# PantoMatrix/PantoMatrix

Hardware: NVIDIA H100
Metric: motion_frames_per_sec (higher is better)
Workload: dtype fp16x3 (two fp16 operand planes, 3 products, f32 accumulate)

## Files before the change

### include/pm_emage.h

```cpp
#ifndef PM_EMAGE_H
#define PM_EMAGE_H
#include <stdint.h>
#ifdef __cplusplus
extern "C" {
#endif

#define PM_ABI_VERSION 6
#define PM_FMT_F16 0x100
#define PM_TC_TILE_SHIFT 16
#define PM_TC_STORE_LOOP (1 << 24)
int pm_abi_version(void);
int pm_memset_async(void* ptr, int value, long long bytes, void* stream);
int pm_device_cc(void);

int pm_tapgemm_f32(const float* A, long long a_bs, int lda, int batch, int rows_in, int cin,
                   const float* W, const float* bias, int taps, int stride, int pad,
                   int rows_out, int cout,
                   const float* residual, long long r_bs, int ldr,
                   int act, float slope,
                   float* out, long long o_bs, int ldo, void* stream);

int pm_tapgemm_tc(const uint16_t* A, long long a_ps, long long a_bs, int lda, int batch, int rows_in, int cin,
                  const uint16_t* W, long long w_ps, int w_rows, int ldw, int taps, int pad, int nsplit,
                  const float* bias, int rows_out, int cout,
                  const float* residual, long long r_bs, int ldr,
                  int act, int act_cols, float slope, float acc_scale,
                  float* out_f32, long long o_bs, int ldo,
                  uint16_t* out_bf16, long long ob_ps, long long ob_bs, int ldob, int out_nsplit,
                  const void* prefetch, long long prefetch_bytes, void* stream);

int pm_split_bf16(const float* x, long long x_bs, int ldx, int batch, int rows, int ch,
                  uint16_t* out, long long o_ps, long long o_bs, int ldo, int nsplit, void* stream);

int pm_wav_stem_f32(const float* audio, long long a_bs, long long a_ws, int batch, int windows, int n_samples,
                    const float* w1, const float* b1, const float* wd, const float* bd, int cout,
                    int ksize, int stride, int pad, int rows_out, float slope,
                    float* y1, float* sc,
                    uint16_t* planes, long long p_ps, int p_ld, int p_nsplit, void* stream);

int pm_add_layernorm_f32(const float* x, const float* r, const float* gamma, const float* beta,
                         float* out, long long rows, int ch, float eps,
                         uint16_t* planes, long long p_ps, int p_ld, int p_nsplit, void* stream);

// ... 110 lines not shown
```

### pantomatrix_b200/csrc/pm_tapgemm_tc.cu

```cuda
#include <cuda.h>
#include <stdio.h>
#include <stdlib.h>

#include <cstring>
#include <type_traits>
#include "pm_common.cuh"
#include "../../include/pm_emage.h"


namespace {

constexpr int BM = 128;
constexpr int BK = 64;
constexpr int MMA_K = 16;
constexpr int A_TILE_BYTES = BM * BK * 2;
constexpr int PRODUCER_THREADS = 128;
constexpr int CONSUMER_THREADS = 256;
constexpr int NUM_THREADS = PRODUCER_THREADS + CONSUMER_THREADS;
constexpr int PRODUCER_REGS = 40, CONSUMER_REGS = 232;
static_assert(PRODUCER_THREADS * PRODUCER_REGS + CONSUMER_THREADS * CONSUMER_REGS == (65536 / NUM_THREADS & ~7) * NUM_THREADS,
              "the setmaxnreg split must use exactly the launch's register pool");
constexpr int STAMP_WARP = PRODUCER_THREADS / 32;
constexpr int MAX_STAGES = 8;
constexpr int RING_KB = 200;

struct TcParams {
  int taps, pad, nsplit, kblocks;
  int rows_out, cout, batch;
  int R, NB;
  int w_rows;
  const float* bias;
  const float* residual; long long r_bs; int ldr;
  int res_tma;
  int tma_out;
  int act, act_cols; float slope;
  float* out_f32; long long o_bs; int ldo;
  __nv_bfloat16* out_bf16; long long ob_ps, ob_bs; int ldob; int out_nsplit;
  int stages;
  int res_slot0, rot;
  const uint8_t* prefetch; long long prefetch_bytes;
  float acc_scale;
};

#ifdef PM_TC_TIMING
__device__ unsigned long long pm_tc_stamps[4096 * 8];
#define PM_STAMP(i)                                                                                              \
  do {                                                                                                           \
    if ((threadIdx.x & 31) == 0) {                                                                               \
      const unsigned cta_ = (blockIdx.z * gridDim.y + blockIdx.y) * gridDim.x + blockIdx.x;                      \
      if (cta_ < 4096) pm_tc_stamps[cta_ * 8 + (i)] = (unsigned long long)clock64();                             \
    }                                                                                                            \
  } while (0)
#else
#define PM_STAMP(i) do {} while (0)
#endif

#include "pm_tc_ptx.cuh"

template <int BN, bool F16>
__device__ __forceinline__ void mma_k16(float (&d)[BN / 2], uint64_t a, uint64_t b) {
  static_assert(BN == 64 || BN == 128, "64- or 128-column tiles (see pm_tapgemm_tc)");
  if constexpr (BN == 64) wgmma_m64n64k16<!F16>(d, a, b);
  else wgmma_m64n128k16<!F16>(d, a, b);
}

template <int BN, bool F16, int NSPLIT>
__device__ __forceinline__ void mma_kblock(float (&main)[BN / 2], float (&corr)[BN / 2], uint64_t a0, uint64_t w0) {
  constexpr uint64_t A_PL = A_TILE_BYTES >> 4, W_PL = (BN * BK * 2) >> 4, K_ST = (MMA_K * 2) >> 4;
  if constexpr (NSPLIT == 3) {
#pragma unroll
    for (int k = 0; k < BK / MMA_K; ++k) mma_k16<BN, F16>(corr, a0 + k * K_ST, w0 + 2 * W_PL + k * K_ST);
#pragma unroll
    for (int k = 0; k < BK / MMA_K; ++k) mma_k16<BN, F16>(corr, a0 + A_PL + k * K_ST, w0 + W_PL + k * K_ST);
#pragma unroll
    for (int k = 0; k < BK / MMA_K; ++k) mma_k16<BN, F16>(corr, a0 + 2 * A_PL + k * K_ST, w0 + k * K_ST);
  }
  if constexpr (NSPLIT >= 2) {
#pragma unroll
    for (int k = 0; k < BK / MMA_K; ++k) mma_k16<BN, F16>(corr, a0 + k * K_ST, w0 + W_PL + k * K_ST);
#pragma unroll
    for (int k = 0; k < BK / MMA_K; ++k) mma_k16<BN, F16>(corr, a0 + A_PL + k * K_ST, w0 + k * K_ST);
  }
#pragma unroll
  for (int k = 0; k < BK / MMA_K; ++k) mma_k16<BN, F16>(main, a0 + k * K_ST, w0 + k * K_ST);
}

template <int BN, bool F16, int NSPLIT>
__global__ void __launch_bounds__(NUM_THREADS, 1) tapgemm_tc_kernel(const __grid_constant__ CUtensorMap map_a,
                                                                  const __grid_constant__ CUtensorMap map_w,
                                                                  const __grid_constant__ CUtensorMap map_r,
                                                                  const __grid_constant__ CUtensorMap map_o,
                                                                  const __grid_constant__ CUtensorMap map_p,
                                                                  const TcParams p) {
  constexpr int W_TILE_BYTES = BN * BK * 2;
  constexpr int NACC = BN / 2;
  constexpr int ST = BN + 8;
  constexpr int RES_BYTES = BM * BN * 4;

  extern __shared__ __align__(1024) uint8_t smem_raw[];
  uint8_t* tiles = smem_raw + ((1024u - (smem_u32(smem_raw) & 1023u)) & 1023u);
  const int stage_bytes = p.nsplit * (A_TILE_BYTES + W_TILE_BYTES);
  const int ring_bytes = p.stages * stage_bytes > BM * ST * 4 ? p.stages * stage_bytes : BM * ST * 4;
  uint64_t* bars = reinterpret_cast<uint64_t*>(tiles + ring_bytes);
  uint64_t* full_bar = bars;
  uint64_t* empty_bar = bars + MAX_STAGES;
  uint64_t* epi_bar = bars + 2 * MAX_STAGES;
  float* bias_s = reinterpret_cast<float*>(bars + 2 * MAX_STAGES + 2);

  const int warp = threadIdx.x >> 5, lane = threadIdx.x & 31;
  if (warp == STAMP_WARP) PM_STAMP(0);
  const int l0 = blockIdx.x * p.R;
  const int n0 = blockIdx.y * BN;
  const int b0 = blockIdx.z * p.NB;
  const int n_iter = p.taps * p.kblocks;

  if (threadIdx.x == 0) {
    asm volatile("prefetch.tensormap [%0];" ::"l"(&map_a) : "memory");
    asm volatile("prefetch.tensormap [%0];" ::"l"(&map_w) : "memory");
    if (p.res_tma) asm volatile("prefetch.tensormap [%0];" ::"l"(&map_r) : "memory");
    if (p.tma_out && p.out_f32) asm volatile("prefetch.tensormap [%0];" ::"l"(&map_o) : "memory");
    if (p.tma_out && p.out_nsplit) asm volatile("prefetch.tensormap [%0];" ::"l"(&map_p) : "memory");
    for (int s = 0; s < p.stages; ++s) {
      mbar_init(smem_u32(&full_bar[s]), 1);
      mbar_init(smem_u32(&empty_bar[s]), 2);
    }
    mbar_init(smem_u32(epi_bar), p.res_tma ? 2 : 1);
    asm volatile("fence.mbarrier_init.release.cluster;" ::: "memory");
  }
  __syncthreads();
  if (warp == STAMP_WARP) PM_STAMP(1);

  if (warp < PRODUCER_THREADS / 32) {
    setmaxnreg_dec<PRODUCER_REGS>();
    if (warp == 1 && lane == 0 && p.prefetch) {
      const long long ncta = (long long)gridDim.x * gridDim.y * gridDim.z;
      const long long cta = ((long long)blockIdx.z * gridDim.y + blockIdx.y) * gridDim.x + blockIdx.x;
      long long share = ((p.prefetch_bytes + ncta - 1) / ncta + 127) & ~127LL;
      long long off = cta * share;
      long long end = off + share < p.prefetch_bytes ? off + share : p.prefetch_bytes;
      end &= ~15LL;
      for (; off < end; off += 16384) {
        const uint32_t n = (uint32_t)(end - off < 16384 ? end - off : 16384);
        asm volatile("cp.async.bulk.prefetch.L2.global [%0], %1;" ::"l"(p.prefetch + off), "r"(n) : "memory");
      }
    }
    if (warp == 2) {
      for (int c = lane; c < BN; c += 32) bias_s[c] = p.bias && n0 + c < p.cout ? __ldg(p.bias + n0 + c) : 0.f;
      __syncwarp();
      if (lane == 0) mbar_arrive(smem_u32(epi_bar));
    }
    if (warp != 0) return;
    const uint32_t tx = (uint32_t)stage_bytes;
    int s = 0, q = p.rot, tap = 0, kb = 0;
    uint32_t ph = 0;
    for (int it = 0; it < n_iter; ++it) {
      mbar_wait_fast(smem_u32(&empty_bar[s]), ph ^ 1u);
      if (elect_one()) {
        const uint32_t bar = smem_u32(&full_bar[s]);
        uint8_t* st = tiles + (size_t)q * stage_bytes;
        mbar_expect_tx(bar, tx);
        for (int pl = 0; pl < p.nsplit; ++pl) {
          tma_load_4d(smem_u32(st + pl * A_TILE_BYTES), &map_a, bar, kb * BK, l0 + tap - p.pad, b0, pl);
          tma_load_3d(smem_u32(st + p.nsplit * A_TILE_BYTES + pl * W_TILE_BYTES), &map_w, bar, kb * BK, tap * p.w_rows + n0, pl);
        }
      }
      __syncwarp();
      if (++s == p.stages) { s = 0; ph ^= 1u; }
      if (++q == p.stages) q = 0;
      if (++kb == p.kblocks) { kb = 0; ++tap; }
    }
    if (p.res_tma) {
      for (int j = p.res_slot0; j < p.stages; ++j) {
        mbar_wait_fast(smem_u32(&empty_bar[s]), ph ^ 1u);
        if (++s == p.stages) { s = 0; ph ^= 1u; }
      }
      if (elect_one()) {
        const uint32_t bar = smem_u32(epi_bar);
        mbar_expect_tx(bar, (uint32_t)RES_BYTES);
        const int nbox = p.tma_out ? BN / 32 : 1;
        for (int j = 0; j < nbox; ++j)
          tma_load_3d(smem_u32(tiles + ring_bytes - RES_BYTES + j * (RES_BYTES / nbox)), &map_r, bar, n0 + j * (BN / nbox), l0, b0);
      }
      __syncwarp();
    }
    return;
  }

  setmaxnreg_inc<CONSUMER_REGS>();
  const int ct = threadIdx.x - PRODUCER_THREADS;
  const int wg = ct >> 7;
  float acc0[NACC], acc1[NACC], accc[NACC];
#pragma unroll
  for (int i = 0; i < NACC; ++i) { acc0[i] = 0.f; acc1[i] = 0.f; accc[i] = 0.f; }
  {
    const uint32_t tiles_u32 = smem_u32(tiles);
    int s = 0, q = p.rot;
    uint32_t ph = 0;
    int prev = -1;
    auto kblock = [&](float (&main)[NACC]) {
      mbar_wait_fast(smem_u32(&full_bar[s]), ph);
      if (prev < 0 && warp == STAMP_WARP) PM_STAMP(2);
      const uint32_t a_base = tiles_u32 + (uint32_t)q * (uint32_t)stage_bytes + (uint32_t)wg * (64 * 128);
      const uint32_t w_base = tiles_u32 + (uint32_t)q * (uint32_t)stage_bytes + (uint32_t)(NSPLIT * A_TILE_BYTES);
      wgmma_fence();
      mma_kblock<BN, F16, NSPLIT>(main, accc, gmma_desc(GMMA_DESC_K_SW128, a_base), gmma_desc(GMMA_DESC_K_SW128, w_base));
      wgmma_commit();
      wgmma_wait<1>();
      if (prev >= 0 && ct % 128 == 0) mbar_arrive(smem_u32(&empty_bar[prev]));
      prev = s;
      if (++s == p.stages) { s = 0; ph ^= 1u; }
      if (++q == p.stages) q = 0;
    };
    int it = 0;
    for (; it + 1 < n_iter; it += 2) {
      kblock(acc0);
      kblock(acc1);
    }
    if (it < n_iter) kblock(acc0);
    if (warp == STAMP_WARP) PM_STAMP(3);
    wgmma_wait<0>();
    if (warp == STAMP_WARP) PM_STAMP(4);
    wgmma_fence_regs(acc0);
    wgmma_fence_regs(acc1);
    wgmma_fence_regs(accc);
  }
  named_bar_sync(1, CONSUMER_THREADS);
  if (p.tma_out) {
    const int wq = warp & 3, t4 = lane & 3, sw = lane >> 2;
    const int r0 = wg * 64 + wq * 16 + sw;
    const float act_slope = p.act == PM_ACT_NONE ? 1.f : (p.act == PM_ACT_RELU ? 0.f : p.slope);
    const float* res_s = reinterpret_cast<const float*>(tiles + ring_bytes - RES_BYTES);
    auto off32 = [&](int r, int i) { return (i >> 2) * (BM * 32) + r * 32 + (((2 * (i & 3) + (t4 >> 1)) ^ sw) << 2) + 2 * (t4 & 1); };
    mbar_wait_fast(smem_u32(epi_bar), 0);
#pragma unroll
    for (int i = 0; i < NACC / 4; ++i) {
      const int c = 8 * i + 2 * t4, n = n0 + c;
      const float2 bc = *reinterpret_cast<const float2*>(bias_s + c);
#pragma unroll
      for (int h = 0; h < 2; ++h) {
        const int j = 4 * i + 2 * h;
        float v0 = acc0[j] + acc1[j], v1 = acc0[j + 1] + acc1[j + 1];
        v0 += accc[j];
        v1 += accc[j + 1];
        if constexpr (F16) { v0 = __fmul_rn(v0, p.acc_scale); v1 = __fmul_rn(v1, p.acc_scale); }
// ... 133 lines not shown
}

template <bool VEC, bool F16>
__global__ void __launch_bounds__(256) split_bf16_kernel(const float* __restrict__ x, long long x_bs, int ldx, int rows,
                                                         int ch, __nv_bfloat16* __restrict__ out, long long o_ps,
                                                         long long o_bs, int ldo, int nsplit) {
  const int b = blockIdx.y;
  const float* __restrict__ xb = x + (long long)b * x_bs;
  __nv_bfloat16* __restrict__ ob = out + (long long)b * o_bs;
  if (VEC) {
    const int ch4 = ch >> 2;
    const long long total = (long long)rows * ch4;
    for (long long i = (long long)blockIdx.x * blockDim.x + threadIdx.x; i < total; i += (long long)gridDim.x * blockDim.x) {
      const int r = (int)(i / ch4), c4 = (int)(i - (long long)r * ch4);
      const float4 v = *reinterpret_cast<const float4*>(xb + (long long)r * ldx + 4 * c4);
      const PmPlanes P{ob, o_ps, ldo, nsplit};
      pm_store_planes4_t<F16>(P, r, 4 * c4, v);
    }
  } else {
    const long long total = (long long)rows * ch;
    for (long long i = (long long)blockIdx.x * blockDim.x + threadIdx.x; i < total; i += (long long)gridDim.x * blockDim.x) {
      const int r = (int)(i / ch), c = (int)(i - (long long)r * ch);
      const PmPlanes P{ob, o_ps, ldo, nsplit};
      pm_store_planes_t<F16>(P, r, c, xb[(long long)r * ldx + c]);
    }
  }
}

constexpr int stage_bytes_of(int bn, int nsplit) { return nsplit * (A_TILE_BYTES + bn * BK * 2); }
constexpr int stages_of(int bn, int nsplit) {
  return RING_KB * 1024 / stage_bytes_of(bn, nsplit) < MAX_STAGES ? RING_KB * 1024 / stage_bytes_of(bn, nsplit) : MAX_STAGES;
}
constexpr int ring_bytes_of(int bn, int nsplit) { return stages_of(bn, nsplit) * stage_bytes_of(bn, nsplit); }
constexpr bool tma_out_fits(int bn, int nsplit, bool f32, int out_nsplit, bool residual) {
  return (f32 ? BM * bn * 4 : 0) + out_nsplit * BM * bn * 2 + (residual ? BM * bn * 4 : 0) <= ring_bytes_of(bn, nsplit);
}

template <int BN, bool F16, int NSPLIT>
int launch(const CUtensorMap& ma, const CUtensorMap& mw, const CUtensorMap& mr, const CUtensorMap& mo,
           const CUtensorMap& mp, TcParams& p, dim3 grid, cudaStream_t st) {
  constexpr int stage_bytes = stage_bytes_of(BN, NSPLIT);
  constexpr int stages = stages_of(BN, NSPLIT);
  static_assert(stages >= 2, "the operand ring needs two stages");
  constexpr int staging = BM * (BN + 8) * 4, res_bytes = BM * BN * 4;
  static_assert(staging + res_bytes <= stages * stage_bytes && res_bytes <= (stages - 1) * stage_bytes,
                "staging and residual tiles must fit the ring side by side");
  static_assert(tma_out_fits(BN, NSPLIT, true, 2, true), "fp32, two plane and residual tiles must fit the ring");
  static_assert(BN * 4 * BM % 1024 == 0 && stage_bytes % 1024 == 0, "128B-swizzled TMA boxes need 1024-byte alignment");
  p.stages = stages;
  p.res_slot0 = (stages * stage_bytes - res_bytes) / stage_bytes;
  p.rot = (p.res_slot0 - 1 - (p.taps * p.kblocks - 1) % stages + stages) % stages;
  const size_t smem = (size_t)stages * stage_bytes + 1024  + (2 * MAX_STAGES + 2) * sizeof(uint64_t) + BN * sizeof(float);
  static unsigned long long configured = 0;
  if (pm_first_use_on_device(configured)) {
    cudaError_t e = cudaFuncSetAttribute(tapgemm_tc_kernel<BN, F16, NSPLIT>, cudaFuncAttributeMaxDynamicSharedMemorySize, 227 * 1024);
    if (e != cudaSuccess) { configured = 0; return (int)e; }
  }
  tapgemm_tc_kernel<BN, F16, NSPLIT><<<grid, NUM_THREADS, smem, st>>>(ma, mw, mr, mo, mp, p);
  PM_LAUNCH_CHECK();
}

template <int BN>
int launch_fmt(const CUtensorMap* m, TcParams& p, dim3 grid, cudaStream_t st, bool f16) {
  if (f16) {
    if (p.nsplit == 1) return launch<BN, true, 1>(m[0], m[1], m[2], m[3], m[4], p, grid, st);
    if (p.nsplit == 2) return launch<BN, true, 2>(m[0], m[1], m[2], m[3], m[4], p, grid, st);
    return launch<BN, true, 3>(m[0], m[1], m[2], m[3], m[4], p, grid, st);
  }
  if (p.nsplit == 1) return launch<BN, false, 1>(m[0], m[1], m[2], m[3], m[4], p, grid, st);
  if (p.nsplit == 2) return launch<BN, false, 2>(m[0], m[1], m[2], m[3], m[4], p, grid, st);
  return launch<BN, false, 3>(m[0], m[1], m[2], m[3], m[4], p, grid, st);
}

int pick_bn(long long row_tiles, int cout, int w_rows, int sms) {
  if (cout <= 64 || w_rows % 128) return 64;
  const long long waves64 = (row_tiles * pm_cdiv(cout, 64) + sms - 1) / sms;
  const long long waves128 = (row_tiles * pm_cdiv(cout, 128) + sms - 1) / sms;
  return waves128 * 14 <= waves64 * 10 ? 128 : 64;
}

}

extern "C" int pm_tapgemm_tc(const uint16_t* A, long long a_ps, long long a_bs, int lda, int batch, int rows_in, int cin,
                             const uint16_t* W, long long w_ps, int w_rows, int ldw, int taps, int pad, int nsplit,
                             const float* bias, int rows_out, int cout,
                             const float* residual, long long r_bs, int ldr,
                             int act, int act_cols, float slope, float acc_scale,
                             float* out_f32, long long o_bs, int ldo,
                             uint16_t* out_bf16, long long ob_ps, long long ob_bs, int ldob, int out_nsplit,
                             const void* prefetch, long long prefetch_bytes, void* stream) {
  PM_REQUIRE(A && W && (out_f32 || out_bf16));
  const int tile = (nsplit >> PM_TC_TILE_SHIFT) & 0xff;
  const bool store_loop = (nsplit & PM_TC_STORE_LOOP) != 0;
  PM_TAKE_FMT(nsplit, f16);
  PM_TAKE_FMT(out_nsplit, out_f16);
  PM_REQUIRE(!out_bf16 || out_f16 == f16);
  PM_REQUIRE(f16 || acc_scale == 1.0f);
  PM_REQUIRE(!prefetch || (prefetch_bytes >= 0 && (reinterpret_cast<uintptr_t>(prefetch) & 15) == 0));
  PM_REQUIRE(batch > 0 && rows_in > 0 && rows_out > 0 && cin > 0 && cout > 0 && taps > 0);
  PM_REQUIRE(nsplit >= 1 && nsplit <= 3 && (!out_bf16 || (out_nsplit >= 1 && out_nsplit <= 3)));
  PM_REQUIRE(act >= PM_ACT_NONE && act <= PM_ACT_LEAKY);
  PM_REQUIRE((reinterpret_cast<uintptr_t>(A) & 15) == 0 && (reinterpret_cast<uintptr_t>(W) & 15) == 0);
  PM_REQUIRE((lda & 7) == 0 && (ldw & 7) == 0 && lda >= cin && ldw >= cin && w_rows >= cout);
  PM_REQUIRE(batch == 1 || (a_bs & 7) == 0);
  PM_REQUIRE(nsplit == 1 || ((a_ps & 7) == 0 && (w_ps & 7) == 0));
  PM_REQUIRE(!out_f32 || ldo >= cout);
  PM_REQUIRE(!out_bf16 || ldob >= cout);
  PM_REQUIRE(!residual || ldr >= cout);

  int R = 128;
  if (rows_out <= 64 && batch > 1) { R = 16; while (R < rows_out) R <<= 1; }
  const int NB = 128 / R;
  PM_REQUIRE(tile <= 2 && w_rows % 64 == 0 && (tile != 2 || w_rows % 128 == 0));
  int BNsel = tile == 1 ? 64 : 128;
  if (tile == 0) {
    int dev = 0, sms = 0;
    cudaError_t e = cudaGetDevice(&dev);
    if (e == cudaSuccess) e = cudaDeviceGetAttribute(&sms, cudaDevAttrMultiProcessorCount, dev);
    if (e != cudaSuccess) return (int)e;
    BNsel = pick_bn((long long)pm_cdiv(rows_out, R) * pm_cdiv(batch, NB), cout, w_rows, sms);
  }

  TcParams p;
  p.taps = taps; p.pad = pad; p.nsplit = nsplit; p.kblocks = (cin + BK - 1) / BK;
  p.rows_out = rows_out; p.cout = cout; p.batch = batch; p.R = R; p.NB = NB; p.w_rows = w_rows;
  p.bias = bias; p.residual = residual; p.r_bs = r_bs; p.ldr = ldr;
  p.act = act; p.act_cols = act_cols <= 0 ? cout : act_cols; p.slope = slope;
  p.out_f32 = out_f32; p.o_bs = o_bs; p.ldo = ldo;
  p.out_bf16 = reinterpret_cast<__nv_bfloat16*>(out_bf16); p.ob_ps = ob_ps; p.ob_bs = ob_bs; p.ldob = ldob;
  p.out_nsplit = out_bf16 ? out_nsplit : 0;
  p.stages = 0;
  p.prefetch = static_cast<const uint8_t*>(prefetch);
  p.prefetch_bytes = prefetch ? prefetch_bytes : 0;
  p.acc_scale = acc_scale;
  CUtensorMap m[5];
  std::memset(m, 0, sizeof(m));
  CUtensorMap &ma = m[0], &mw = m[1], &mr = m[2], &mo = m[3], &mp = m[4];
  {
    const long long bs_el = batch > 1 ? a_bs : (long long)rows_in * lda;
    const long long ps_el = nsplit > 1 ? a_ps : bs_el * batch;
    cuuint64_t dims[4] = {(cuuint64_t)cin, (cuuint64_t)rows_in, (cuuint64_t)batch, (cuuint64_t)nsplit};
    cuuint64_t strides[3] = {(cuuint64_t)lda * 2, (cuuint64_t)bs_el * 2, (cuuint64_t)ps_el * 2};
    cuuint32_t box[4] = {(cuuint32_t)BK, (cuuint32_t)R, (cuuint32_t)NB, 1};
    if (!encode_map(&ma, A, 4, dims, strides, box, f16)) return PM_EBADARG;
  }
  {
    const long long ps_el = nsplit > 1 ? w_ps : (long long)taps * w_rows * ldw;
    cuuint64_t dims[3] = {(cuuint64_t)cin, (cuuint64_t)taps * w_rows, (cuuint64_t)nsplit};
    cuuint64_t strides[2] = {(cuuint64_t)ldw * 2, (cuuint64_t)ps_el * 2};
    cuuint32_t box[3] = {(cuuint32_t)BK, (cuuint32_t)BNsel, 1};
    if (!encode_map(&mw, W, 3, dims, strides, box, f16)) return PM_EBADARG;
  }
  const bool res_ok = residual && (reinterpret_cast<uintptr_t>(residual) & 15) == 0 && (ldr & 3) == 0 && (batch == 1 || (r_bs & 3) == 0);
  bool tma_out = !store_loop && (!residual || res_ok) && tma_out_fits(BNsel, nsplit, out_f32, p.out_nsplit, residual);
  if (tma_out && out_f32) {
    tma_out = (reinterpret_cast<uintptr_t>(out_f32) & 15) == 0 && (ldo & 3) == 0 && (batch == 1 || (o_bs & 3) == 0);
    const long long bs_el = batch > 1 ? o_bs : (long long)rows_out * ldo;
    cuuint64_t dims[3] = {(cuuint64_t)cout, (cuuint64_t)rows_out, (cuuint64_t)batch};
    cuuint64_t strides[2] = {(cuuint64_t)ldo * 4, (cuuint64_t)bs_el * 4};
    cuuint32_t box[3] = {32, (cuuint32_t)R, (cuuint32_t)NB};
    tma_out = tma_out && encode_tiled(&mo, CU_TENSOR_MAP_DATA_TYPE_FLOAT32, CU_TENSOR_MAP_SWIZZLE_128B, out_f32, 3, dims, strides, box);
  }
  if (tma_out && out_bf16) {
    tma_out = (reinterpret_cast<uintptr_t>(out_bf16) & 15) == 0 && (ldob & 7) == 0 && (batch == 1 || (ob_bs & 7) == 0) &&
              (out_nsplit == 1 || (ob_ps & 7) == 0);
    const long long bs_el = batch > 1 ? ob_bs : (long long)rows_out * ldob;
    const long long ps_el = out_nsplit > 1 ? ob_ps : bs_el * batch;
    cuuint64_t dims[4] = {(cuuint64_t)cout, (cuuint64_t)rows_out, (cuuint64_t)batch, (cuuint64_t)out_nsplit};
    cuuint64_t strides[3] = {(cuuint64_t)ldob * 2, (cuuint64_t)bs_el * 2, (cuuint64_t)ps_el * 2};
    cuuint32_t box[4] = {64, (cuuint32_t)R, (cuuint32_t)NB, 1};
    tma_out = tma_out && encode_map(&mp, out_bf16, 4, dims, strides, box, f16);
  }
  p.res_tma = false;
  for (int swz = tma_out; res_ok && !p.res_tma && swz >= 0; --swz) {
    const long long bs_el = batch > 1 ? r_bs : (long long)rows_out * ldr;
    cuuint64_t dims[3] = {(cuuint64_t)cout, (cuuint64_t)rows_out, (cuuint64_t)batch};
    cuuint64_t strides[2] = {(cuuint64_t)ldr * 4, (cuuint64_t)bs_el * 4};
    cuuint32_t box[3] = {swz ? 32u : (cuuint32_t)BNsel, (cuuint32_t)R, (cuuint32_t)NB};
    p.res_tma = encode_tiled(&mr, CU_TENSOR_MAP_DATA_TYPE_FLOAT32, swz ? CU_TENSOR_MAP_SWIZZLE_128B : CU_TENSOR_MAP_SWIZZLE_NONE,
                             residual, 3, dims, strides, box);
    if (!p.res_tma) tma_out = false;
  }
  p.tma_out = tma_out;
  dim3 grid(pm_cdiv(rows_out, R), pm_cdiv(cout, BNsel), pm_cdiv(batch, NB));
  PM_REQUIRE(grid.z <= 65535 && grid.y <= 65535);
  const cudaStream_t st = (cudaStream_t)stream;
  if (BNsel == 128) return launch_fmt<128>(m, p, grid, st, f16);
// ... 44 lines not shown
```

### pantomatrix_b200/emage_audio/engine.py

```python
from __future__ import annotations

import os

import torch

from .. import ops

PARTS = ("face", "upper", "hands", "lower")
WAV_BLOCKS = ((5, 1600, True), (6, 0, True), (1, 7, False), (6, 0, True), (1, 7, False), (3, 0, True))
NHEAD = 4


def _taps(w: torch.Tensor) -> torch.Tensor:
    return w.permute(2, 0, 1).contiguous()


def _fold_bn(sd, conv, bn, eps=1e-5):
    w, b = sd[conv + ".weight"].double(), sd[conv + ".bias"].double()
    s = sd[bn + ".weight"].double() / torch.sqrt(sd[bn + ".running_var"].double() + eps)
    return (w * s[:, None, None]).float(), ((b - sd[bn + ".running_mean"].double()) * s + sd[bn + ".bias"].double()).float()


def wav_out_len(n: int) -> int:
    length = n
# ... 95 lines not shown
            _record_stream(results[i], cur)
        return results


class _Conv:
    __slots__ = ("w", "b", "stride", "pad", "_packed", "_next")

    def __init__(self, w, b, stride=1, pad=0):
        self.w, self.b, self.stride, self.pad = w, b, stride, pad
        self._packed = {}
        self._next = None

    def _prefetch_hint(self, ns):
        prev = _STATE.get("prev_conv")
        if prev is not None and prev is not self:
            prev._next = self
        _STATE["prev_conv"] = self
        nxt = self._next
        return nxt._packed[_pk(ns)].t if (nxt is not None and _pk(ns) in nxt._packed) else None

    def packed(self, nsplit):
        key = _pk(nsplit)
        if key not in self._packed:
            w, s = self.w, self.stride
            if s > 1:
                taps, cout, cin = w.shape
                wp = torch.zeros(-(-taps // s), cout, s * cin, device=w.device, dtype=w.dtype)
                for k in range(taps):
                    wp[k // s, :, (k % s) * cin:(k % s + 1) * cin] = w[k]
                w = wp
            self._packed[key] = ops.PackedW(w, nsplit)
        return self._packed[key]

    def __call__(self, x, act=ops.ACT_NONE, slope=0.0, residual=None, out=None, want="f", out_slack=0):
        ns = _STATE["nsplit"]
        residual = _f32(residual)
        if ns == 0:
            y = ops.tapgemm(_f32(x), self.w, self.b, stride=self.stride, pad=self.pad, act=act, slope=slope,
                            residual=residual, out=out)
            return y if want == "f" else ops.Act(y, None)
        taps, cout, _ = self.w.shape
        s = self.stride
        want_f, out_ns = "f" in want, (ns if "p" in want else 0)
        pf = self._prefetch_hint(ns)
        if s == 1:
            a = _planes(x, ns)
            batch, rows = a.batch, a.rows
            rows_out = rows + 2 * self.pad - taps + 1
            flat = (taps == 1 and batch > 1 and a.t.stride(1) == rows * a.t.stride(2)
                    and (out is None or out.is_contiguous()) and (residual is None or residual.is_contiguous()))
            if want_f and out is None:
                out = torch.empty(batch, rows_out, cout, device=a.t.device, dtype=torch.float32)
            if flat:
                _, pl = ops.tapgemm_tc(a.flat(), self.packed(ns), self.b, rows_out=batch * rows, act=act, slope=slope,
                                       want_f32=want_f, out=None if out is None else out.view(1, batch * rows, cout),
                                       residual=None if residual is None else residual.view(1, batch * rows, cout),
                                       out_nsplit=out_ns, out_slack=out_slack, prefetch=pf)
                if pl is not None:
                    pl = ops.Planes(pl.t.view(pl.t.shape[0], batch, rows, pl.t.shape[3]), rows, cout, pl.slack)
            else:
                _, pl = ops.tapgemm_tc(a, self.packed(ns), self.b, rows_out=rows_out, pad=self.pad, act=act, slope=slope,
                                       residual=residual, want_f32=want_f, out=out, out_nsplit=out_ns, out_slack=out_slack,
                                       prefetch=pf)
            return out if want == "f" else ops.Act(out, pl)
        assert self.pad == 0
        a = _planes(x, ns, need_slack=s)
        batch, rows, cin = a.batch, a.rows, a.ch
        assert a.t.stride(2) == cin and a.t.stride(1) == rows * cin, "strided view needs dense (clips*rows, C) planes"
        rows_out = (rows - taps) // s + 1
        o, pl = ops.tapgemm_tc(a, self.packed(ns), self.b, rows_out=rows_out, act=act, slope=slope, residual=residual,
                               want_f32=want_f, out=out, out_nsplit=out_ns, out_slack=out_slack, prefetch=pf,
                               a_view=(-(-rows // s), s * cin, s * cin))
        return o if want == "f" else ops.Act(o, pl)


def _f32(x):
    if isinstance(x, ops.Act):
        assert x.f is not None, "this consumer needs the fp32 copy"
        return x.f
    return x


def _planes(x, ns, need_slack=0):
    if isinstance(x, ops.Planes):
        assert x.slack >= need_slack
        return x
    if isinstance(x, ops.Act):
        if x.p is not None and x.p.nsplit == ns and x.p.slack >= need_slack and x.p.t.dtype == ops._PLANE_DTYPE:
            return x.p
        x = x.f
    return ops.split_bf16(x, ns, slack_rows=need_slack)


def _ns():
    return _STATE["nsplit"]


class _Linear(_Conv):
    def __init__(self, sd, prefix=None, w=None, b=None):
        if prefix is not None:
            w, b = sd[prefix + ".weight"], sd[prefix + ".bias"]
        super().__init__(w.contiguous().unsqueeze(0), None if b is None else b.contiguous())

# ... 20 lines not shown
            self.steps.append(("res", c(0, ".model.0"), c(0, ".model.2")))
            self.steps.append(("res", c(1, ".model.0"), c(1, ".model.2")))
            for i in range(n_layer):
                self.steps.append(("conv", c(2 + 2 * i), True))
            self.steps.append(("conv", c(2 + 2 * n_layer), False))

    def __call__(self, x, want="f"):
        last = len(self.steps) - 1
        for i, step in enumerate(self.steps):
            w = want if i == last else "fp"
            if step[0] == "conv":
                x = step[1](x, act=ops.ACT_LEAKY if step[2] else ops.ACT_NONE, slope=0.2, want=w)
            else:
                x = step[2](step[1](x, act=ops.ACT_LEAKY, slope=0.2, want="p"), residual=x, want=w)
        return x


class _WavEncoder:

    def __init__(self, sd, p, blocks=WAV_BLOCKS):
        self.blocks = []
        for i, (stride, pad, has_ds) in enumerate(blocks):
            q = f"{p}.feat_extractor.{i}"
            w1, b1 = _fold_bn(sd, q + ".conv1", q + ".bn1")
            w2, b2 = _fold_bn(sd, q + ".conv2", q + ".bn2")
            ds = _fold_bn(sd, q + ".downsample.0", q + ".downsample.1") if has_ds else None
            if i == 0:
                self.stem = (w1.reshape(w1.shape[0], -1).contiguous(), b1.contiguous(),
                             ds[0].reshape(ds[0].shape[0], -1).contiguous(), ds[1].contiguous(), stride, pad)
                self.blocks.append((None, _Conv(_taps(w2), b2.contiguous(), 1, 7), None))
            else:
                self.blocks.append((_Conv(_taps(w1), b1.contiguous(), stride, pad), _Conv(_taps(w2), b2.contiguous(), 1, 7),
                                    _Conv(_taps(ds[0]), ds[1].contiguous(), stride, pad) if ds else None))

    def __call__(self, audio, offset, a_ws, windows, n_samples, out=None):
        bs, n = audio.shape
        w1, b1, wd, bd, stride, pad = self.stem
        y, sc = ops.wav_stem(audio, n, a_ws, bs, windows, n_samples, w1, b1, wd, bd, stride=stride, pad=pad,
                             slope=0.01, offset=offset, nsplit=_ns())
        last = len(self.blocks) - 1
        form = lambda i: "f" if i == last else ("p" if self.blocks[i + 1][2] is not None else "fp")
        x = self.blocks[0][1](y, act=ops.ACT_LEAKY, slope=0.01, residual=sc, want=form(0), out_slack=8)
        for i, (conv1, conv2, ds) in enumerate(self.blocks[1:], 1):
            y = conv1(x, act=ops.ACT_LEAKY, slope=0.01, want="p")
            sc = ds(x) if ds is not None else x
            x = conv2(y, act=ops.ACT_LEAKY, slope=0.01, residual=sc, want=form(i), out_slack=8,
                      out=out if i == last else None)
        return x


class _Attn:

    def __init__(self, sd, p, E):
        w, b = sd[p + ".in_proj_weight"], sd[p + ".in_proj_bias"]
        self.qkv = _Linear(None, w=w, b=b)
        self.q = _Linear(None, w=w[:E], b=b[:E])
        self.kv = _Linear(None, w=w[E:], b=b[E:])
        self.out = _Linear(sd, p + ".out_proj")
        self.E = E


class _Layer:

    def __init__(self, sd, p, E, cross):
        self.E = E
        self.sa = _Attn(sd, p + ".self_attn", E)
        self.ca = _Attn(sd, p + ".multihead_attn", E) if cross else None
        self.l1, self.l2 = _Linear(sd, p + ".linear1"), _Linear(sd, p + ".linear2")
        n = 3 if cross else 2
        self.norms = [(sd[f"{p}.norm{i + 1}.weight"].contiguous(), sd[f"{p}.norm{i + 1}.bias"].contiguous()) for i in range(n)]

    def project_memory(self, mem):
        return self.ca.kv(mem, want="p" if _attn_tc() else "f")

    def __call__(self, x, mem_kv=None, want="f"):
        ns = _ns()
        xf = _f32(x)
        bs, t, E = xf.shape
# ... 289 lines not shown
```

### pantomatrix_b200/ops.py

```python
from __future__ import annotations

import math

import torch

from . import _lib

ACT_NONE, ACT_RELU, ACT_LEAKY = 0, 1, 2
ROW_NONE, ROW_PE, ROW_SPK = 0, 1, 2

launch_count = 0

FMT_F16 = 0x100
TC_TILE_SHIFT = 16
TC_STORE_LOOP = 1 << 24
F16_ACT_SCALE = 64.0
_PLANE_DTYPE = torch.bfloat16


def set_plane_format(name: str) -> None:
    global _PLANE_DTYPE
    _PLANE_DTYPE = {"bf16": torch.bfloat16, "fp16": torch.float16}[name]


def plane_format() -> str:
    return "fp16" if _PLANE_DTYPE == torch.float16 else "bf16"


def _fmt_bit(t) -> int:
    return FMT_F16 if t.dtype == torch.float16 else 0


def _stream() -> int:
    return torch.cuda.current_stream().cuda_stream


def _ptr(t) -> int | None:
    return None if t is None else t.data_ptr()


def _chk(t: torch.Tensor, dtype=torch.float32):
    if not t.is_cuda:
        raise _lib.PmError("pantomatrix_b200 ops need CUDA tensors (no CPU fallback)")
    if t.dtype != dtype:
        raise _lib.PmError(f"expected {dtype}, got {t.dtype}")
    if t.dim() and t.stride(-1) != 1 and t.shape[-1] != 1:
        raise _lib.PmError("innermost dimension must be contiguous")
    return t
# ... 363 lines not shown
    _call("pm_split_bf16", x.data_ptr(), x_bs, ldx, batch, rows, ch, pl.t.data_ptr(), pl.t.stride(0), pl.t.stride(1),
          pl.t.stride(2), nsplit | _fmt_bit(pl.t), _stream())
    return pl


class PackedW:
    __slots__ = ("t", "taps", "cout", "cin", "w_rows", "ldw", "acc_scale")

    def __init__(self, w, nsplit):
        taps, cout, cin = w.shape
        bn = 64 if cout <= 64 else 128
        self.taps, self.cout, self.cin = taps, cout, cin
        self.w_rows, self.ldw = _round_up(cout, bn), _round_up(cin, 8)
        full = torch.zeros(taps, self.w_rows, self.ldw, device=w.device, dtype=torch.float32)
        full[:, :cout, :cin] = w
        self.acc_scale = 1.0
        if _PLANE_DTYPE == torch.float16:
            m = float(full.abs().max())
            if m > 0.0 and math.isfinite(m):
                k = math.floor(math.log2(32768.0 / m))
                full = full * (2.0 ** k)
                self.acc_scale = 2.0 ** -k
            self.acc_scale /= F16_ACT_SCALE
        planes, rem = [], full
        for _ in range(nsplit):
            p = rem.to(_PLANE_DTYPE)
            planes.append(p)
            rem = rem - p.float()
        self.t = torch.stack(planes).contiguous()


def tapgemm_tc(a: Planes, w: PackedW, bias, *, rows_in=None, rows_out, pad=0, act=ACT_NONE, act_cols=0, slope=0.0,
               residual=None, want_f32=True, out_nsplit=0, out=None, a_view=None, out_slack=0, prefetch=None, tile=0,
               store_loop=False):
    t = a.t
    nsplit, batch = t.shape[0], t.shape[1]
    assert nsplit == w.t.shape[0] and t.dtype == w.t.dtype, "A and W must use the same split and plane format"
    fmt = _fmt_bit(t)
    rows_a, cin, lda = (a.rows, a.ch, t.stride(2)) if a_view is None else a_view
    if rows_in is not None:
        rows_a = rows_in
    assert cin == w.cin, (cin, w.cin)
    assert tile in (0, 64, 128), tile
    cout = w.cout
    dev = t.device
    out_f = None
    if want_f32:
        out_f = out if out is not None else torch.empty(batch, rows_out, cout, device=dev, dtype=torch.float32)
        assert out_f.shape == (batch, rows_out, cout)
    o_bs, ldo = _bs_ld(out_f) if out_f is not None else (0, 0)
    out_p = None
    if out_nsplit:
        out_p = _new_planes(out_nsplit, (batch, rows_out), cout, dev, out_slack, dtype=t.dtype)
    r_bs, ldr = _bs_ld(residual) if residual is not None else (0, 0)
    if residual is not None:
        _chk(residual)
        assert residual.shape == (batch, rows_out, cout)
    _call("pm_tapgemm_tc", t.data_ptr(), t.stride(0), t.stride(1), lda, batch, rows_a, cin,
          w.t.data_ptr(), w.t.stride(0), w.w_rows, w.ldw, w.taps, pad, nsplit | fmt | (tile // 64) << TC_TILE_SHIFT | (TC_STORE_LOOP if store_loop else 0),
          _ptr(bias), rows_out, cout, _ptr(residual), r_bs, ldr, act, act_cols, float(slope), float(w.acc_scale),
          _ptr(out_f), o_bs, ldo,
          None if out_p is None else out_p.t.data_ptr(), 0 if out_p is None else out_p.t.stride(0),
          0 if out_p is None else out_p.t.stride(1), 0 if out_p is None else out_p.t.stride(2),
          out_nsplit | (fmt if out_nsplit else 0),
          None if prefetch is None else prefetch.data_ptr(),
          0 if prefetch is None else prefetch.numel() * prefetch.element_size(), _stream())
    return out_f, out_p




def lstm_bidir(xproj, whh, barrier, hidden):
    _chk(xproj), _chk(whh)
    assert xproj.is_contiguous() and whh.is_contiguous() and whh.shape == (2, 4 * hidden, hidden)
    batch, t, w = xproj.shape
    assert w == 8 * hidden
    y = torch.empty(batch, t, 2 * hidden, device=xproj.device, dtype=torch.float32)
    _call("pm_lstm_bidir_f32", xproj.data_ptr(), xproj.stride(0), xproj.stride(1), whh.data_ptr(), y.data_ptr(),
          y.stride(0), y.stride(1), barrier.data_ptr(), batch, t, hidden, _stream())
    return y


def rot6d_to_aa(rot6d, slot, n_sel):
    _chk(rot6d)
    assert rot6d.is_contiguous() and rot6d.shape[-1] == n_sel * 6
    rows = rot6d.numel() // (n_sel * 6)
    out = torch.empty(*rot6d.shape[:-1], 165, device=rot6d.device, dtype=torch.float32)
    _call("pm_rot6d_to_aa_f32", rot6d.data_ptr(), rows, n_sel, slot.data_ptr(), out.data_ptr(), _stream())
    return out



# ... 163 lines not shown
```

Before: 340,500.

## Load A halo once per tile for multi-tap convs and fuse conv1 with downsample

For tap convolutions with few k-blocks, the producer now loads one A halo region (BM+taps-1 rows) per k-block into shared memory, and each tap reads it through a shifted descriptor offset. Previously every tap reloaded a full A tile. This cuts A traffic by roughly a factor of taps, but leaves less shared memory for W pipeline stages. Separately, the audio encoder concatenates the conv1 and downsample weights into one GEMM when their scales match, with the activation applied only to the conv1 columns, which saves a launch and a second read of the input.

```diff
diff --git a/include/pm_emage.h b/include/pm_emage.h
--- a/include/pm_emage.h
+++ b/include/pm_emage.h
@@ -9,6 +9,7 @@
 #define PM_FMT_F16 0x100
 #define PM_TC_TILE_SHIFT 16
 #define PM_TC_STORE_LOOP (1 << 24)
+#define PM_TC_NO_HALO (1 << 25)
 int pm_abi_version(void);
 int pm_memset_async(void* ptr, int value, long long bytes, void* stream);
 int pm_device_cc(void);
diff --git a/pantomatrix_b200/csrc/pm_tapgemm_tc.cu b/pantomatrix_b200/csrc/pm_tapgemm_tc.cu
--- a/pantomatrix_b200/csrc/pm_tapgemm_tc.cu
+++ b/pantomatrix_b200/csrc/pm_tapgemm_tc.cu
@@ -37,6 +37,9 @@
   float* out_f32; long long o_bs; int ldo;
   __nv_bfloat16* out_bf16; long long ob_ps, ob_bs; int ldob; int out_nsplit;
   int stages;
+  int ring0;
+  int halo_rows;
+  int halo_plane;
   int res_slot0, rot;
   const uint8_t* prefetch; long long prefetch_bytes;
   float acc_scale;
@@ -65,8 +68,9 @@
 }
 
 template <int BN, bool F16, int NSPLIT>
-__device__ __forceinline__ void mma_kblock(float (&main)[BN / 2], float (&corr)[BN / 2], uint64_t a0, uint64_t w0) {
-  constexpr uint64_t A_PL = A_TILE_BYTES >> 4, W_PL = (BN * BK * 2) >> 4, K_ST = (MMA_K * 2) >> 4;
+__device__ __forceinline__ void mma_kblock(float (&main)[BN / 2], float (&corr)[BN / 2], uint64_t a0, uint64_t w0,
+                                           uint64_t A_PL) {
+  constexpr uint64_t W_PL = (BN * BK * 2) >> 4, K_ST = (MMA_K * 2) >> 4;
   if constexpr (NSPLIT == 3) {
 #pragma unroll
     for (int k = 0; k < BK / MMA_K; ++k) mma_k16<BN, F16>(corr, a0 + k * K_ST, w0 + 2 * W_PL + k * K_ST);
@@ -85,7 +89,7 @@
   for (int k = 0; k < BK / MMA_K; ++k) mma_k16<BN, F16>(main, a0 + k * K_ST, w0 + k * K_ST);
 }
 
-template <int BN, bool F16, int NSPLIT>
+template <int BN, bool F16, int NSPLIT, bool HALO>
 __global__ void __launch_bounds__(NUM_THREADS, 1) tapgemm_tc_kernel(const __grid_constant__ CUtensorMap map_a,
                                                                   const __grid_constant__ CUtensorMap map_w,
                                                                   const __grid_constant__ CUtensorMap map_r,
@@ -99,13 +103,17 @@
 
   extern __shared__ __align__(1024) uint8_t smem_raw[];
   uint8_t* tiles = smem_raw + ((1024u - (smem_u32(smem_raw) & 1023u)) & 1023u);
-  const int stage_bytes = p.nsplit * (A_TILE_BYTES + W_TILE_BYTES);
-  const int ring_bytes = p.stages * stage_bytes > BM * ST * 4 ? p.stages * stage_bytes : BM * ST * 4;
+  constexpr bool halo = HALO;
+  const int w_off = halo ? 0 : p.nsplit * A_TILE_BYTES;
+  const int stage_bytes = p.nsplit * W_TILE_BYTES + w_off;
+  const int ring0 = halo ? p.ring0 : 0;
+  const int ring_bytes = ring0 + p.stages * stage_bytes > BM * ST * 4 ? ring0 + p.stages * stage_bytes : BM * ST * 4;
   uint64_t* bars = reinterpret_cast<uint64_t*>(tiles + ring_bytes);
   uint64_t* full_bar = bars;
   uint64_t* empty_bar = bars + MAX_STAGES;
   uint64_t* epi_bar = bars + 2 * MAX_STAGES;
-  float* bias_s = reinterpret_cast<float*>(bars + 2 * MAX_STAGES + 2);
+  uint64_t* halo_bar = bars + 2 * MAX_STAGES + 1;
+  float* bias_s = reinterpret_cast<float*>(bars + 2 * MAX_STAGES + 4);
 
   const int warp = threadIdx.x >> 5, lane = threadIdx.x & 31;
   if (warp == STAMP_WARP) PM_STAMP(0);
@@ -125,6 +133,8 @@
       mbar_init(smem_u32(&empty_bar[s]), 2);
     }
     mbar_init(smem_u32(epi_bar), p.res_tma ? 2 : 1);
+    if (halo)
+      for (int kb = 0; kb < p.kblocks; ++kb) mbar_init(smem_u32(&halo_bar[kb]), 1);
     asm volatile("fence.mbarrier_init.release.cluster;" ::: "memory");
   }
   __syncthreads();
@@ -151,18 +161,28 @@
     }
     if (warp != 0) return;
     const uint32_t tx = (uint32_t)stage_bytes;
+    auto load_halo = [&](int k) {
+      const uint32_t bar = smem_u32(&halo_bar[k]);
+      mbar_expect_tx(bar, (uint32_t)(p.nsplit * p.halo_rows * BK * 2));
+      for (int pl = 0; pl < p.nsplit; ++pl)
+        tma_load_4d(smem_u32(tiles + (k * p.nsplit + pl) * p.halo_plane), &map_a, bar, k * BK, l0 - p.pad, b0, pl);
+    };
+    if (halo && elect_one()) load_halo(0);
+    __syncwarp();
     int s = 0, q = p.rot, tap = 0, kb = 0;
     uint32_t ph = 0;
     for (int it = 0; it < n_iter; ++it) {
       mbar_wait_fast(smem_u32(&empty_bar[s]), ph ^ 1u);
       if (elect_one()) {
         const uint32_t bar = smem_u32(&full_bar[s]);
-        uint8_t* st = tiles + (size_t)q * stage_bytes;
+        uint8_t* st = tiles + ring0 + (size_t)q * stage_bytes;
         mbar_expect_tx(bar, tx);
         for (int pl = 0; pl < p.nsplit; ++pl) {
-          tma_load_4d(smem_u32(st + pl * A_TILE_BYTES), &map_a, bar, kb * BK, l0 + tap - p.pad, b0, pl);
-          tma_load_3d(smem_u32(st + p.nsplit * A_TILE_BYTES + pl * W_TILE_BYTES), &map_w, bar, kb * BK, tap * p.w_rows + n0, pl);
+          if (!halo) tma_load_4d(smem_u32(st + pl * A_TILE_BYTES), &map_a, bar, kb * BK, l0 + tap - p.pad, b0, pl);
+          tma_load_3d(smem_u32(st + w_off + pl * W_TILE_BYTES), &map_w, bar, kb * BK, tap * p.w_rows + n0, pl);
         }
+        if (halo && it == 0)
+          for (int k = 1; k < p.kblocks; ++k) load_halo(k);
       }
       __syncwarp();
       if (++s == p.stages) { s = 0; ph ^= 1u; }
@@ -194,22 +214,27 @@
   for (int i = 0; i < NACC; ++i) { acc0[i] = 0.f; acc1[i] = 0.f; accc[i] = 0.f; }
   {
     const uint32_t tiles_u32 = smem_u32(tiles);
-    int s = 0, q = p.rot;
+    const uint64_t a_pl = (uint64_t)(halo ? p.halo_plane : A_TILE_BYTES) >> 4;
+    int s = 0, q = p.rot, tap = 0, kb = 0;
     uint32_t ph = 0;
     int prev = -1;
     auto kblock = [&](float (&main)[NACC]) {
+      if (halo && tap == 0) mbar_wait_fast(smem_u32(&halo_bar[kb]), 0);
       mbar_wait_fast(smem_u32(&full_bar[s]), ph);
       if (prev < 0 && warp == STAMP_WARP) PM_STAMP(2);
-      const uint32_t a_base = tiles_u32 + (uint32_t)q * (uint32_t)stage_bytes + (uint32_t)wg * (64 * 128);
-      const uint32_t w_base = tiles_u32 + (uint32_t)q * (uint32_t)stage_bytes + (uint32_t)(NSPLIT * A_TILE_BYTES);
+      const uint32_t st = tiles_u32 + (uint32_t)ring0 + (uint32_t)q * (uint32_t)stage_bytes;
+      const uint32_t a_base = halo ? tiles_u32 + (uint32_t)(kb * NSPLIT * p.halo_plane) + (uint32_t)(64 * wg + tap) * 128u
+                                   : st + (uint32_t)wg * (64 * 128);
+      const uint32_t w_base = st + (uint32_t)w_off;
       wgmma_fence();
-      mma_kblock<BN, F16, NSPLIT>(main, accc, gmma_desc(GMMA_DESC_K_SW128, a_base), gmma_desc(GMMA_DESC_K_SW128, w_base));
+      mma_kblock<BN, F16, NSPLIT>(main, accc, gmma_desc(GMMA_DESC_K_SW128, a_base), gmma_desc(GMMA_DESC_K_SW128, w_base), a_pl);
       wgmma_commit();
       wgmma_wait<1>();
       if (prev >= 0 && ct % 128 == 0) mbar_arrive(smem_u32(&empty_bar[prev]));
       prev = s;
       if (++s == p.stages) { s = 0; ph ^= 1u; }
       if (++q == p.stages) q = 0;
+      if (++kb == p.kblocks) { kb = 0; ++tap; }
     };
     int it = 0;
     for (; it + 1 < n_iter; it += 2) {
@@ -409,8 +434,20 @@
   return RING_KB * 1024 / stage_bytes_of(bn, nsplit) < MAX_STAGES ? RING_KB * 1024 / stage_bytes_of(bn, nsplit) : MAX_STAGES;
 }
 constexpr int ring_bytes_of(int bn, int nsplit) { return stages_of(bn, nsplit) * stage_bytes_of(bn, nsplit); }
-constexpr bool tma_out_fits(int bn, int nsplit, bool f32, int out_nsplit, bool residual) {
-  return (f32 ? BM * bn * 4 : 0) + out_nsplit * BM * bn * 2 + (residual ? BM * bn * 4 : 0) <= ring_bytes_of(bn, nsplit);
+constexpr int halo_plane_of(int taps) { return ((BM + taps - 1) * BK * 2 + 1023) & ~1023; }
+constexpr int halo_bytes_of(int nsplit, int kblocks, int taps) { return kblocks * nsplit * halo_plane_of(taps); }
+constexpr int halo_stages_of(int bn, int nsplit, int kblocks, int taps) {
+  return (RING_KB * 1024 - halo_bytes_of(nsplit, kblocks, taps)) / (nsplit * bn * BK * 2) < MAX_STAGES
+             ? (RING_KB * 1024 - halo_bytes_of(nsplit, kblocks, taps)) / (nsplit * bn * BK * 2) : MAX_STAGES;
+}
+constexpr int operand_bytes_of(int bn, int nsplit, bool halo) { return halo ? RING_KB * 1024 : ring_bytes_of(bn, nsplit); }
+constexpr bool tma_out_fits(int bn, int nsplit, bool halo, bool f32, int out_nsplit, bool residual) {
+  return (f32 ? BM * bn * 4 : 0) + out_nsplit * BM * bn * 2 + (residual ? BM * bn * 4 : 0) <= operand_bytes_of(bn, nsplit, halo);
+}
+constexpr bool halo_fits(int bn, int nsplit, int kblocks, int taps) {
+  return BM + taps - 1 <= 256 && halo_stages_of(bn, nsplit, kblocks, taps) >= 2 &&
+         BM * bn * 4 <= (halo_stages_of(bn, nsplit, kblocks, taps) - 1) * nsplit * bn * BK * 2 &&
+         BM * (bn + 8) * 4 + BM * bn * 4 <= RING_KB * 1024 && tma_out_fits(bn, nsplit, true, true, 2, true);
 }
 
 template <int BN, bool F16, int NSPLIT>
@@ -422,18 +459,28 @@
   constexpr int staging = BM * (BN + 8) * 4, res_bytes = BM * BN * 4;
   static_assert(staging + res_bytes <= stages * stage_bytes && res_bytes <= (stages - 1) * stage_bytes,
                 "staging and residual tiles must fit the ring side by side");
-  static_assert(tma_out_fits(BN, NSPLIT, true, 2, true), "fp32, two plane and residual tiles must fit the ring");
+  static_assert(tma_out_fits(BN, NSPLIT, false, true, 2, true), "fp32, two plane and residual tiles must fit the ring");
   static_assert(BN * 4 * BM % 1024 == 0 && stage_bytes % 1024 == 0, "128B-swizzled TMA boxes need 1024-byte alignment");
-  p.stages = stages;
-  p.res_slot0 = (stages * stage_bytes - res_bytes) / stage_bytes;
-  p.rot = (p.res_slot0 - 1 - (p.taps * p.kblocks - 1) % stages + stages) % stages;
-  const size_t smem = (size_t)stages * stage_bytes + 1024  + (2 * MAX_STAGES + 2) * sizeof(uint64_t) + BN * sizeof(float);
-  static unsigned long long configured = 0;
-  if (pm_first_use_on_device(configured)) {
-    cudaError_t e = cudaFuncSetAttribute(tapgemm_tc_kernel<BN, F16, NSPLIT>, cudaFuncAttributeMaxDynamicSharedMemorySize, 227 * 1024);
-    if (e != cudaSuccess) { configured = 0; return (int)e; }
-  }
-  tapgemm_tc_kernel<BN, F16, NSPLIT><<<grid, NUM_THREADS, smem, st>>>(ma, mw, mr, mo, mp, p);
+  static_assert(halo_fits(BN, NSPLIT, 1, 15) && halo_fits(BN, NSPLIT, 2, 15) == !(BN == 128 && NSPLIT == 3),
+                "the k = 15 convs' halo regions must fit the operand region beside two W stages");
+  static_assert((NSPLIT * BN * BK * 2) % 1024 == 0, "halo mode: 1024-aligned W stages");
+  const int ws = NSPLIT * BN * BK * 2;
+  p.stages = p.halo_rows ? halo_stages_of(BN, NSPLIT, p.kblocks, p.taps) : stages;
+  const int sb = p.halo_rows ? ws : stage_bytes;
+  p.ring0 = p.halo_rows ? RING_KB * 1024 - p.stages * ws : 0;
+  p.halo_plane = p.halo_rows ? halo_plane_of(p.taps) : 0;
+  p.res_slot0 = (p.stages * sb - res_bytes) / sb;
+  p.rot = (p.res_slot0 - 1 - (p.taps * p.kblocks - 1) % p.stages + p.stages) % p.stages;
+  const size_t smem = (size_t)operand_bytes_of(BN, NSPLIT, p.halo_rows != 0) + 1024  +
+                      (2 * MAX_STAGES + 4) * sizeof(uint64_t) + BN * sizeof(float);
+  const bool halo = p.halo_rows != 0;
+  const auto kernel = halo ? tapgemm_tc_kernel<BN, F16, NSPLIT, true> : tapgemm_tc_kernel<BN, F16, NSPLIT, false>;
+  static unsigned long long configured[2] = {0, 0};
+  if (pm_first_use_on_device(configured[halo])) {
+    cudaError_t e = cudaFuncSetAttribute(kernel, cudaFuncAttributeMaxDynamicSharedMemorySize, 227 * 1024);
+    if (e != cudaSuccess) { configured[halo] = 0; return (int)e; }
+  }
+  kernel<<<grid, NUM_THREADS, smem, st>>>(ma, mw, mr, mo, mp, p);
   PM_LAUNCH_CHECK();
 }
 
@@ -469,6 +516,7 @@
   PM_REQUIRE(A && W && (out_f32 || out_bf16));
   const int tile = (nsplit >> PM_TC_TILE_SHIFT) & 0xff;
   const bool store_loop = (nsplit & PM_TC_STORE_LOOP) != 0;
+  const bool no_halo = (nsplit & PM_TC_NO_HALO) != 0;
   PM_TAKE_FMT(nsplit, f16);
   PM_TAKE_FMT(out_nsplit, out_f16);
   PM_REQUIRE(!out_bf16 || out_f16 == f16);
@@ -507,6 +555,8 @@
   p.out_bf16 = reinterpret_cast<__nv_bfloat16*>(out_bf16); p.ob_ps = ob_ps; p.ob_bs = ob_bs; p.ldob = ldob;
   p.out_nsplit = out_bf16 ? out_nsplit : 0;
   p.stages = 0;
+  const bool halo = !no_halo && taps >= 3 && R == BM && p.kblocks <= 2 && halo_fits(BNsel, nsplit, p.kblocks, taps);
+  p.halo_rows = halo ? R + taps - 1 : 0;
   p.prefetch = static_cast<const uint8_t*>(prefetch);
   p.prefetch_bytes = prefetch ? prefetch_bytes : 0;
   p.acc_scale = acc_scale;
@@ -518,7 +568,7 @@
     const long long ps_el = nsplit > 1 ? a_ps : bs_el * batch;
     cuuint64_t dims[4] = {(cuuint64_t)cin, (cuuint64_t)rows_in, (cuuint64_t)batch, (cuuint64_t)nsplit};
     cuuint64_t strides[3] = {(cuuint64_t)lda * 2, (cuuint64_t)bs_el * 2, (cuuint64_t)ps_el * 2};
-    cuuint32_t box[4] = {(cuuint32_t)BK, (cuuint32_t)R, (cuuint32_t)NB, 1};
+    cuuint32_t box[4] = {(cuuint32_t)BK, (cuuint32_t)(halo ? p.halo_rows : R), (cuuint32_t)NB, 1};
     if (!encode_map(&ma, A, 4, dims, strides, box, f16)) return PM_EBADARG;
   }
   {
@@ -529,7 +579,7 @@
     if (!encode_map(&mw, W, 3, dims, strides, box, f16)) return PM_EBADARG;
   }
   const bool res_ok = residual && (reinterpret_cast<uintptr_t>(residual) & 15) == 0 && (ldr & 3) == 0 && (batch == 1 || (r_bs & 3) == 0);
-  bool tma_out = !store_loop && (!residual || res_ok) && tma_out_fits(BNsel, nsplit, out_f32, p.out_nsplit, residual);
+  bool tma_out = !store_loop && (!residual || res_ok) && tma_out_fits(BNsel, nsplit, halo, out_f32, p.out_nsplit, residual);
   if (tma_out && out_f32) {
     tma_out = (reinterpret_cast<uintptr_t>(out_f32) & 15) == 0 && (ldo & 3) == 0 && (batch == 1 || (o_bs & 3) == 0);
     const long long bs_el = batch > 1 ? o_bs : (long long)rows_out * ldo;
diff --git a/pantomatrix_b200/emage_audio/engine.py b/pantomatrix_b200/emage_audio/engine.py
--- a/pantomatrix_b200/emage_audio/engine.py
+++ b/pantomatrix_b200/emage_audio/engine.py
@@ -151,7 +151,7 @@
             self._packed[key] = ops.PackedW(w, nsplit)
         return self._packed[key]
 
-    def __call__(self, x, act=ops.ACT_NONE, slope=0.0, residual=None, out=None, want="f", out_slack=0):
+    def __call__(self, x, act=ops.ACT_NONE, slope=0.0, residual=None, out=None, want="f", out_slack=0, act_cols=0):
         ns = _STATE["nsplit"]
         residual = _f32(residual)
         if ns == 0:
@@ -187,7 +187,8 @@
         batch, rows, cin = a.batch, a.rows, a.ch
         assert a.t.stride(2) == cin and a.t.stride(1) == rows * cin, "strided view needs dense (clips*rows, C) planes"
         rows_out = (rows - taps) // s + 1
-        o, pl = ops.tapgemm_tc(a, self.packed(ns), self.b, rows_out=rows_out, act=act, slope=slope, residual=residual,
+        o, pl = ops.tapgemm_tc(a, self.packed(ns), self.b, rows_out=rows_out, act=act, act_cols=act_cols, slope=slope,
+                               residual=residual,
                                want_f32=want_f, out=out, out_nsplit=out_ns, out_slack=out_slack, prefetch=pf,
                                a_view=(-(-rows // s), s * cin, s * cin))
         return o if want == "f" else ops.Act(o, pl)
@@ -274,6 +275,24 @@
             else:
                 self.blocks.append((_Conv(_taps(w1), b1.contiguous(), stride, pad), _Conv(_taps(w2), b2.contiguous(), 1, 7),
                                     _Conv(_taps(ds[0]), ds[1].contiguous(), stride, pad) if ds else None))
+        self._pair = {}
+
+    def _conv1_ds(self, i, x):
+        conv1, _, ds = self.blocks[i]
+        ns = _ns()
+        key = (i, _pk(ns)) if ns else None
+        if key is not None and key not in self._pair:
+            pw1, pwd = conv1.packed(ns), ds.packed(ns)
+            same_scale = pw1.acc_scale == pwd.acc_scale and conv1.w.shape == ds.w.shape and conv1.pad == ds.pad
+            self._pair[key] = _Conv(torch.cat([conv1.w, ds.w], 1), torch.cat([conv1.b, ds.b]), conv1.stride,
+                                    conv1.pad) if same_scale else None
+        pair = self._pair.get(key)
+        if pair is None:
+            return conv1(x, act=ops.ACT_LEAKY, slope=0.01, want="p"), ds(x)
+        cout = conv1.w.shape[1]
+        yz = pair(x, act=ops.ACT_LEAKY, slope=0.01, want="fp", act_cols=cout)
+        y = ops.Planes(yz.p.t, yz.p.rows, cout, yz.p.slack)
+        return ops.Act(None, y), yz.f[:, :, cout:]
 
     def __call__(self, audio, offset, a_ws, windows, n_samples, out=None):
         bs, n = audio.shape
@@ -284,8 +303,10 @@
         form = lambda i: "f" if i == last else ("p" if self.blocks[i + 1][2] is not None else "fp")
         x = self.blocks[0][1](y, act=ops.ACT_LEAKY, slope=0.01, residual=sc, want=form(0), out_slack=8)
         for i, (conv1, conv2, ds) in enumerate(self.blocks[1:], 1):
-            y = conv1(x, act=ops.ACT_LEAKY, slope=0.01, want="p")
-            sc = ds(x) if ds is not None else x
+            if ds is not None:
+                y, sc = self._conv1_ds(i, x)
+            else:
+                y, sc = conv1(x, act=ops.ACT_LEAKY, slope=0.01, want="p"), x
             x = conv2(y, act=ops.ACT_LEAKY, slope=0.01, residual=sc, want=form(i), out_slack=8,
                       out=out if i == last else None)
         return x
diff --git a/pantomatrix_b200/ops.py b/pantomatrix_b200/ops.py
--- a/pantomatrix_b200/ops.py
+++ b/pantomatrix_b200/ops.py
@@ -14,6 +14,7 @@
 FMT_F16 = 0x100
 TC_TILE_SHIFT = 16
 TC_STORE_LOOP = 1 << 24
+TC_NO_HALO = 1 << 25
 F16_ACT_SCALE = 64.0
 _PLANE_DTYPE = torch.bfloat16
 
@@ -443,7 +444,7 @@
 
 def tapgemm_tc(a: Planes, w: PackedW, bias, *, rows_in=None, rows_out, pad=0, act=ACT_NONE, act_cols=0, slope=0.0,
                residual=None, want_f32=True, out_nsplit=0, out=None, a_view=None, out_slack=0, prefetch=None, tile=0,
-               store_loop=False):
+               store_loop=False, halo=True):
     t = a.t
     nsplit, batch = t.shape[0], t.shape[1]
     assert nsplit == w.t.shape[0] and t.dtype == w.t.dtype, "A and W must use the same split and plane format"
@@ -468,7 +469,8 @@
         _chk(residual)
         assert residual.shape == (batch, rows_out, cout)
     _call("pm_tapgemm_tc", t.data_ptr(), t.stride(0), t.stride(1), lda, batch, rows_a, cin,
-          w.t.data_ptr(), w.t.stride(0), w.w_rows, w.ldw, w.taps, pad, nsplit | fmt | (tile // 64) << TC_TILE_SHIFT | (TC_STORE_LOOP if store_loop else 0),
+          w.t.data_ptr(), w.t.stride(0), w.w_rows, w.ldw, w.taps, pad, nsplit | fmt | (tile // 64) << TC_TILE_SHIFT | (TC_STORE_LOOP if store_loop else 0)
+          | (0 if halo else TC_NO_HALO),
           _ptr(bias), rows_out, cout, _ptr(residual), r_bs, ldr, act, act_cols, float(slope), float(w.acc_scale),
           _ptr(out_f), o_bs, ldo,
           None if out_p is None else out_p.t.data_ptr(), 0 if out_p is None else out_p.t.stride(0),
```

New measurement: 352,300 (median of 6 runs). 1.03x the previous value.
